# jarrodhroberson/diamond-types

Measured on AMD Instinct MI355X. Metric: merged ops/sec (whole node) for batched checkout, higher is better.
Workload: dtype u32/u8 integer

## Files before the change

diamond-types_amd/csrc/dt_replay.hip:

```cpp
#include <hip/hip_runtime.h>

#include <algorithm>
#include <cstdlib>
#include <stdint.h>

#include "dt_device.hpp"
#include "dt_wave.hpp"

namespace dtgpu {
namespace dev {
using namespace wave;

#define BALLOT(c) __ballot(c)
DEV uint32_t vflag(bool c) {
    uint32_t x = c ? 1u : 0u;
    asm volatile("" : "+v"(x));
    return x;
}

constexpr uint32_t BLK = 64;
constexpr uint32_t SBC = 64;
constexpr uint32_t ROOT_ID = 0xFFFFFFFFu;
constexpr uint32_t END_ID = 0xFFFFFFFEu;
constexpr uint32_t NONE = 0xFFFFFFFFu;
constexpr uint32_t C_VIS = 1u, C_LIVE = 1u << 8, C_ITEMS = 1u << 16;
constexpr uint32_t C_UP = 1u << 24;
constexpr uint32_t C_DIRTY = 1u << 31;
DEV uint32_t c_vis(uint32_t c) { return c & 0xFFu; }
DEV uint32_t c_live(uint32_t c) { return (c >> 8) & 0xFFu; }
DEV uint32_t c_items(uint32_t c) { return (c >> 16) & 0xFFu; }
DEV uint32_t c_up(uint32_t c) { return (c >> 24) & 0x7Fu; }
DEV uint32_t pc_blk(uint32_t w) { return w & 0xFFFFu; }
DEV uint32_t pc_cnt(uint32_t w) { return w >> 16; }
DEV uint32_t pc_of(uint32_t b, uint32_t k) { return b | (k << 16); }

template <typename T> DEV T ld(const T *p) { return *p; }
template <typename T> DEV T vld(const T *p) { return *reinterpret_cast<const volatile T *>(p); }
DEV const BatchParams &KP() {
    return *(const BatchParams *)(__builtin_amdgcn_kernarg_segment_ptr());
}
#define GLOBAL_AS __attribute__((address_space(1)))
template <typename T> DEV GLOBAL_AS T *gp(T *p) { return (GLOBAL_AS T *)p; }
template <typename T> DEV void st(T *p, T v) { *p = v; }
template <typename T> DEV T ld_sc(const T *p) { return __hip_atomic_load(p, __ATOMIC_RELAXED, __HIP_MEMORY_SCOPE_WORKGROUP); }
template <typename T> DEV void st_sc(T *p, T v) { __hip_atomic_store(p, v, __ATOMIC_RELAXED, __HIP_MEMORY_SCOPE_WORKGROUP); }
DEV uint32_t cv_add(uint32_t *p, uint32_t d) { return __hip_atomic_fetch_add(p, d, __ATOMIC_RELAXED, __HIP_MEMORY_SCOPE_WORKGROUP); }
template <typename T> DEV void at_xor(T *p, T v) { __hip_atomic_fetch_xor(p, v, __ATOMIC_RELAXED, __HIP_MEMORY_SCOPE_WORKGROUP); }
template <typename T> DEV void at_add(T *p, T v) { __hip_atomic_fetch_add(p, v, __ATOMIC_RELAXED, __HIP_MEMORY_SCOPE_WORKGROUP); }
template <typename T> DEV void at_or(T *p, T v) { __hip_atomic_fetch_or(p, v, __ATOMIC_RELAXED, __HIP_MEMORY_SCOPE_WORKGROUP); }

template <int L> DEV uint32_t ix(const uint32_t *p) {
    if (L) return *p;
    return ld_sc(p);
}
template <int L> DEV uint32_t ix16(const uint16_t *p) { return *p; }

enum ProfSlot { P_INS = 0, P_DEL, P_TOG, P_MAT, P_YJS, P_SPLIT, P_FIND, P_BLOAD, P_ORR, P_RUN, P_R1, P_R2, P_R3, P_N_YJS, P_N_SPLIT,
                P_T1, P_T2, P_T3, P_N_DIRTY, P_N_LOAD, P_N_LOOK, P_N_SKIP, P_N };

struct Doc {
    const Cmd *cmds;
    uint32_t ncmd, n_lv;
    const uint32_t *tlist;
    const DocDesc *desc;
    uint32_t *pc;
    u64 *ao;
    uint32_t *items;
    u64 *m2;
    uint32_t max_blocks, max_sb;
    uint32_t *cnt, *opos;
    uint16_t *opos16;
    uint32_t *sbn, *sbpos;
    uint32_t *top, *tlive;
    uint16_t *sbl;
    uint32_t nb, nsb;
    uint32_t err;
    uint32_t debug;
    uint32_t site;
    uint32_t steps;
    uint64_t prof[P_N];
    uint32_t doc;
    uint32_t cb, cit;
    u64 cmv, cml;
    uint32_t cpre, cpos;
    u64 *mup;
    uint32_t *tup;
    uint32_t *xf;
};

constexpr uint32_t PRE_NONE = 0x80000000u;
DEV bool pre_known(uint32_t pre) { return int32_t(pre) >= 0; }

DEV void fail(Doc &D, uint32_t code, uint32_t site) {
    if (!D.err) { D.err = code; D.site = site; }
}
DEV bool charge(Doc &D) {
    if (D.steps == 0) { fail(D, ErrCapacity, 1); return false; }
    D.steps--;
    return true;
}
template <bool PROF> DEV uint64_t tick() { return PROF ? __builtin_amdgcn_s_memtime() : 0; }

constexpr int IX_HBM = 0, IX_LDS = 1, IX_FLAT = 2;
template <int L> DEV uint32_t opos_of(const Doc &D, uint32_t b) {
    if (L) return D.opos16[b];
    return ix<L>(D.opos + b);
}
template <int L> DEV void set_opos(Doc &D, uint32_t b, uint32_t v) {
    if (L) D.opos16[b] = uint16_t(v);
    else D.opos[b] = v;
}


template <int L> DEV uint32_t first_block(const Doc &D) {
    if (L == IX_FLAT) return U(D.sbl[0]);
    return U(ix16<L>(D.sbl + size_t(U(ix<L>(D.top)) >> 16) * SBC));
}
template <int L> DEV uint32_t next_block(const Doc &D, uint32_t b) {
    if (L == IX_FLAT) {
        const uint32_t p = U(D.opos16[b]) + 1;
        return p < D.nb ? U(D.sbl[p]) : NONE;
    }
    const uint32_t o = U(opos_of<L>(D, b));
    const uint32_t S = o >> 6, i = o & 63u;
    if (i + 1 < U(ix<L>(D.sbn + S))) return U(ix16<L>(D.sbl + size_t(S) * SBC + i + 1));
    const uint32_t p = U(ix<L>(D.sbpos + S)) + 1;
    if (p >= D.nsb) return NONE;
    return U(ix16<L>(D.sbl + size_t(U(ix<L>(D.top + p)) >> 16) * SBC));
}
template <int L> DEV uint32_t key_at(const Doc &D, uint32_t b, uint32_t s) {
    if (L == IX_FLAT) return (uint32_t(D.opos16[b]) << 6) | s;
    const uint32_t o = opos_of<L>(D, b);
    return (ix<L>(D.sbpos + (o >> 6)) << 12) | ((o & 63u) << 6) | s;
}
DEV uint32_t find_slot(const Doc &D, uint32_t b, uint32_t item) {
    const uint4 *row = reinterpret_cast<const uint4 *>(D.items + size_t(b) * BLK);
    uint32_t s = BLK;
    for (uint32_t q = 0; q < BLK / 4 && s == BLK; q += 2) {
        uint4 v[2];
#pragma unroll
        for (uint32_t j = 0; j < 2; j++) v[j] = row[q + j];
#pragma unroll
        for (int j = 1; j >= 0; j--) {
            const uint32_t o = 4 * (q + uint32_t(j));
            if (v[j].w == item) s = o + 3;
            if (v[j].z == item) s = o + 2;
            if (v[j].y == item) s = o + 1;
            if (v[j].x == item) s = o;
        }
    }
    return s;
}
template <int L> DEV uint32_t key_of(const Doc &D, uint32_t item) {
    const uint32_t b = pc_blk(ld(D.pc + item));
    return key_at<L>(D, b, find_slot(D, b, item));
}
template <int L> DEV uint32_t ukey_of(const Doc &D, uint32_t item) {
    const uint32_t b = U(pc_blk(ld(D.pc + item)));
    const u64 m = BALLOT(D.items[size_t(b) * BLK + lane()] == item);
    return U(key_at<L>(D, b, ctz(m)));
}

struct Found {
    uint32_t b, k;
    uint32_t S, tp;
    uint32_t c;
    uint32_t p;
};
template <int L>
DEV bool find_vis(Doc &D, uint32_t p, Found &f) {
    const uint32_t l = lane();
    uint32_t base = 0, S = NONE;
    if (L == IX_FLAT) {
        const uint32_t nc = (D.nb + 63) >> 6;
        {
            const uint32_t w0 = D.top[min(l, nc - 1)];
            const uint32_t v = l < nc ? (w0 & 0xFFFFu) : 0u;
            const uint32_t inc = scan_incl32(v);
            const u64 m = BALLOT(inc > p) & 0xFFFFFFFFull;
            if (!m) return false;
            S = ctz(m);
            base = rdl(inc - v, S);
        }
        f.S = f.tp = S;
        const uint32_t q = (S << 6) + l;
        const uint32_t b0 = D.sbl[min(q, D.nb - 1)];
        const uint32_t w = D.cnt[b0];
        const uint32_t b = q < D.nb ? b0 : 0;
        const uint32_t v = q < D.nb ? c_vis(w) : 0;
        const uint32_t inc = scan_incl(v);
        const u64 m = BALLOT(base + inc > p);
        if (!m) return false;
        const uint32_t fl = ctz(m);
        f.b = U(rdl(b, fl));
        f.k = U(p - base - rdl(inc - v, fl));
        f.c = U(rdl(w, fl));
        f.p = (S << 6) + fl;
        return true;
    }
    for (uint32_t c = 0; c < D.nsb; c += 64) {
        const uint32_t i = c + l;
        const uint32_t w0 = ix<L>(D.top + min(i, D.nsb - 1));
        const uint32_t w = i < D.nsb ? w0 : 0;
        const uint32_t v = w & 0xFFFFu;
        const uint32_t inc = scan_incl(v);
        const u64 m = BALLOT(base + inc > p);
        if (m) {
            const uint32_t fl = ctz(m);
            S = U(rdl(w, fl) >> 16);
            f.tp = U(c + fl);
            base += rdl(inc - v, fl);
            break;
        }
        base += rdl(inc, 63);
    }
    if (S == NONE) return false;
    f.S = S;
    f.c = NONE;
    const uint32_t n = U(ix<L>(D.sbn + S));
    const uint32_t b0 = ix16<L>(D.sbl + size_t(S) * SBC + l);
    const uint32_t b = l < n ? b0 : 0;
    const uint32_t v0 = c_vis(ix<L>(D.cnt + b));
    const uint32_t v = l < n ? v0 : 0;
    const uint32_t inc = scan_incl(v);
    const u64 m = BALLOT(base + inc > p);
    if (!m) return false;
    const uint32_t fl = ctz(m);
    f.b = U(rdl(b, fl));
    f.k = U(p - base - rdl(inc - v, fl));
    return true;
}

DEV uint32_t select_bit(u64 m, uint32_t k) {
    const uint32_t l = lane();
    const bool set = (m >> l) & 1ull;
    const uint32_t before = uint32_t(__popcll(m & lanes_below(l)));
    return ctz(BALLOT(set && before == k));
}

template <int L>
DEV uint32_t next_live_block(Doc &D, uint32_t b) {
    const uint32_t l = lane();
    if (L == IX_FLAT) {
        const uint32_t p0 = U(D.opos16[b]) + 1, nc = (D.nb + 63) >> 6;
        uint32_t c = p0 >> 6;
        {
            const uint32_t q = (c << 6) + l;
            const uint32_t b0 = D.sbl[min(q, D.nb - 1)];
            const bool in = q >= p0 && q < D.nb;
            const uint32_t bl = in ? b0 : 0;
            const uint32_t cl = c_live(D.cnt[bl]);
            const u64 m = BALLOT(in && cl != 0);
            if (m) return U(rdl(bl, ctz(m)));
        }
        for (c = c + 1; c < nc; c += 64) {
            if (!charge(D)) return NONE;
            const uint32_t i = c + l;
            const uint32_t t = D.top[min(i, nc - 1)] >> 16;
            const u64 m = BALLOT(i < nc && t != 0);
            if (m) {
                const uint32_t q = ((c + ctz(m)) << 6) + l;
                const uint32_t b0 = D.sbl[min(q, D.nb - 1)];
                const uint32_t bl = q < D.nb ? b0 : 0;
                const uint32_t cl = c_live(D.cnt[bl]);
                const u64 m2 = BALLOT(q < D.nb && cl != 0);
                if (!m2) { fail(D, ErrCheckout, 19); return NONE; }
                return U(rdl(bl, ctz(m2)));
            }
        }
        return NONE;
    }
    const uint32_t o = U(opos_of<L>(D, b));
    uint32_t S = o >> 6;
    {
        const uint32_t n = U(ix<L>(D.sbn + S)), i0 = (o & 63u) + 1;
        const uint32_t b0 = ix16<L>(D.sbl + size_t(S) * SBC + l);
        const uint32_t bl = l < n ? b0 : 0;
        const uint32_t cl = c_live(ix<L>(D.cnt + bl));
        const u64 m = BALLOT(l >= i0 && l < n && cl != 0);
        if (m) return U(rdl(bl, ctz(m)));
    }
    for (uint32_t p = U(ix<L>(D.sbpos + S)) + 1; p < D.nsb; p += 64) {
        if (!charge(D)) return NONE;
        const uint32_t i = p + l;
        const uint32_t tl = ix<L>(D.tlive + min(i, D.nsb - 1));
        const u64 m = BALLOT(i < D.nsb && tl != 0);
        if (m) {
            S = U(ix<L>(D.top + p + ctz(m)) >> 16);
            const uint32_t n = U(ix<L>(D.sbn + S));
            const uint32_t b0 = ix16<L>(D.sbl + size_t(S) * SBC + l);
            const uint32_t bl = l < n ? b0 : 0;
            const uint32_t cl = c_live(ix<L>(D.cnt + bl));
            const u64 m2 = BALLOT(l < n && cl != 0);
            if (!m2) { fail(D, ErrCheckout, 19); return NONE; }
            return U(rdl(bl, ctz(m2)));
        }
    }
    return NONE;
}


template <int L, bool XF>
DEV void split_sb(Doc &D, uint32_t S) {
    const uint32_t l = lane();
    if (D.nsb >= D.max_sb) { fail(D, ErrCapacity, 21); return; }
    const uint32_t S2 = D.nsb;
    uint32_t vis = 0, live = 0, up = 0;
    {
        const uint32_t b = ix16<L>(D.sbl + size_t(S) * SBC + l);
        const uint32_t c = ix<L>(D.cnt + b);
        vis = c_vis(c);
        live = c_live(c);
        up = c_up(c);
        fence_wave();
        if (l >= SBC / 2) {
            D.sbl[size_t(S2) * SBC + (l - SBC / 2)] = uint16_t(b);
            set_opos<L>(D, b, (S2 << 6) | (l - SBC / 2));
        }
    }
    const uint32_t vh = wave_sum(l >= 32 ? vis : 0), lh = wave_sum(l >= 32 ? live : 0);
    const uint32_t vl = wave_sum(l < 32 ? vis : 0), ll = wave_sum(l < 32 ? live : 0);
    const uint32_t uh = XF ? wave_sum(l >= 32 ? up : 0) : 0, ul = XF ? wave_sum(l < 32 ? up : 0) : 0;
    const uint32_t p = U(ix<L>(D.sbpos + S)) + 1;
    for (int c = int(D.nsb) - 1; c >= int(p); c -= 64) {
        const int i = c - int(l);
        uint32_t w = 0, lv = 0, uv = 0;
        if (i >= int(p)) { w = ix<L>(D.top + i); lv = ix<L>(D.tlive + i); if (XF) uv = ix<L>(D.tup + i); }
        fence_wave();
        if (i >= int(p)) {
            D.top[i + 1] = w; D.tlive[i + 1] = lv; D.sbpos[w >> 16] = uint32_t(i + 1);
            if (XF) D.tup[i + 1] = uv;
        }
        fence_wave();
    }
    if (l == 0) {
        D.sbn[S] = SBC / 2;
        D.sbn[S2] = SBC / 2;
        D.top[p - 1] = (S << 16) | vl; D.tlive[p - 1] = ll;
        D.top[p] = (S2 << 16) | vh; D.tlive[p] = lh;
        D.sbpos[S2] = p;
        if (XF) { D.tup[p - 1] = ul; D.tup[p] = uh; }
    }
    fence_wave();
    D.nsb++;
}

template <int L, bool XF>
DEV uint32_t split_block(Doc &D, uint32_t b, uint32_t c, uint32_t it, u64 mv, u64 ml) {
    const uint32_t l = lane();
    if (D.nb >= D.max_blocks) { fail(D, ErrCapacity, 12); return 0; }
    const uint32_t b2 = D.nb;
    u64 mu = 0, mu_lo = 0, mu_hi = 0;
    if (XF) {
        mu = U64(ld(D.mup + b));
        mu_lo = mu & lanes_below(c);
        mu_hi = c >= 64 ? 0ull : mu >> c;
    }
    if (l >= c) {
        D.items[size_t(b2) * BLK + (l - c)] = it;
        st(D.pc + it, (ld(D.pc + it) & 0xFFFF0000u) | b2);
    }
    const u64 lo = lanes_below(c);
    const u64 mv_hi = c >= 64 ? 0ull : mv >> c, ml_hi = c >= 64 ? 0ull : ml >> c;
    if (l < 4) {
        const u64 v = l == 0 ? (mv & lo) : l == 1 ? (ml & lo) : l == 2 ? mv_hi : ml_hi;
        st(D.m2 + 2 * size_t(l < 2 ? b : b2) + (l & 1), v);
    }
    if (L == IX_FLAT) {
        const uint32_t pos = U(D.opos16[b]);
        for (int hi = int(D.nb) - 1; hi > int(pos); hi -= 64) {
            const int q = hi - int(l);
            const bool mvl = q > int(pos);
            uint32_t v = 0;
            if (mvl) v = D.sbl[q];
            fence_wave();
            if (mvl) {
                D.sbl[q + 1] = uint16_t(v);
                D.opos16[v] = uint16_t(q + 1);
                if (((q + 1) & 63) == 0) {
                    const uint32_t cv = D.cnt[v];
                    const uint32_t w = c_vis(cv) | (c_live(cv) << 16);
                    at_add(D.top + (uint32_t(q) >> 6), 0u - w);
                    at_add(D.top + (uint32_t(q + 1) >> 6), w);
                }
            }
            fence_wave();
        }
        if (l == 0) {
            const uint32_t v2 = uint32_t(__popcll(mv_hi)), l2 = uint32_t(__popcll(ml_hi));
            D.cnt[b2] = v2 * C_VIS + l2 * C_LIVE + (BLK - c) * C_ITEMS;
            D.cnt[b] = uint32_t(__popcll(mv & lo)) * C_VIS + uint32_t(__popcll(ml & lo)) * C_LIVE + c * C_ITEMS;
            D.sbl[pos + 1] = uint16_t(b2);
            D.opos16[b2] = uint16_t(pos + 1);
            if (((pos + 1) & 63) == 0) {
                const uint32_t w = v2 | (l2 << 16);
                at_add(D.top + (pos >> 6), 0u - w);
                at_add(D.top + ((pos + 1) >> 6), w);
            }
        }
        fence_wave();
        D.nb++;
        return b2;
    }
    const uint32_t o = U(opos_of<L>(D, b));
    const uint32_t S = o >> 6, i = o & 63u, n = U(ix<L>(D.sbn + S));
    {
        uint32_t v = 0;
        const bool mv_lane = l > i && l < n;
        if (mv_lane) v = ix16<L>(D.sbl + size_t(S) * SBC + l);
        fence_wave();
        if (mv_lane) {
            D.sbl[size_t(S) * SBC + l + 1] = uint16_t(v);
            set_opos<L>(D, v, (S << 6) | (l + 1));
        }
    }
    if (l == 0) {
        D.cnt[b2] = uint32_t(__popcll(mv_hi)) * C_VIS + uint32_t(__popcll(ml_hi)) * C_LIVE + (BLK - c) * C_ITEMS +
                    uint32_t(__popcll(mu_hi)) * C_UP;
        D.cnt[b] = uint32_t(__popcll(mv & lo)) * C_VIS + uint32_t(__popcll(ml & lo)) * C_LIVE + c * C_ITEMS +
                   uint32_t(__popcll(mu_lo)) * C_UP;
        if (XF) { st(D.mup + b, mu_lo); st(D.mup + b2, mu_hi); }
        D.sbl[size_t(S) * SBC + i + 1] = uint16_t(b2);
        set_opos<L>(D, b2, (S << 6) | (i + 1));
        D.sbn[S] = n + 1;
    }
    fence_wave();
    D.nb++;
    if (n + 1 == SBC) split_sb<L, XF>(D, S);
    return b2;
}

template <int L> DEV uint32_t cut_point(uint32_t s) { return L ? min(max(s, 16u), 48u) : BLK / 2; }

template <int L>
DEV uint32_t up_rank(Doc &D, uint32_t b, uint32_t s) {
    const uint32_t l = lane();
    const uint32_t o = U(opos_of<L>(D, b));
    const uint32_t S = o >> 6, i = o & 63u, tp = U(ix<L>(D.sbpos + S));
    uint32_t r = 0;
    for (uint32_t c = 0; c < tp; c += 64) r += wave_sum(c + l < tp ? ix<L>(D.tup + c + l) : 0u);
    const uint32_t bl = l < i ? ix16<L>(D.sbl + size_t(S) * SBC + l) : 0;
    r += wave_sum(l < i ? c_up(ix<L>(D.cnt + bl)) : 0u);
    r += uint32_t(__popcll(U64(ld(D.mup + b)) & lanes_below(s)));
    return U(r);
}

template <int L, bool PROF, bool XF>
DEV void insert_run(Doc &D, uint32_t b, uint32_t s, uint32_t it, u64 mv, u64 ml, uint32_t lv, uint32_t k,
                    uint32_t ol, uint32_t orr, uint32_t tph, uint32_t c_in) {
    constexpr bool PC = L == IX_FLAT && !XF;
    D.cb = NONE;
    const uint32_t b_in = b;
    const uint32_t l = lane();
    const uint32_t lv0 = lv, k0 = k;
    if (XF) {
        const uint32_t r0 = up_rank<L>(D, b, s);
        for (uint32_t j = l; j < k0; j += 64) D.xf[lv0 + j] = r0 + j;
    }
    if (!XF && c_in != NONE && c_items(c_in) + k <= BLK) {
        const uint32_t shifted = shfl(it, l >= k ? l - k : l);
        it = l < s ? it : (l < s + k ? lv + (l - s) : shifted);
        D.items[size_t(b) * BLK + l] = it;
        if (l >= s && l < s + k) st(D.pc + it, pc_of(b, 1u));
        const u64 low = lanes_below(s);
        const u64 ins = lanes_below(k) << s;
        mv = k == 64 ? ins : ((mv & low) | ((mv & ~low) << k) | ins);
        ml = k == 64 ? ins : ((ml & low) | ((ml & ~low) << k) | ins);
        st(D.m2 + 2 * size_t(b) + (l & 1u), (l & 1u) ? ml : mv);
        if (tph == NONE) tph = L == IX_FLAT ? U(uint32_t(D.opos16[b]) >> 6) : U(ix<L>(D.sbpos + (opos_of<L>(D, b) >> 6)));
        if (l == 0) {
            D.cnt[b] = c_in + k * (C_VIS + C_LIVE + C_ITEMS);
            if (L == IX_FLAT) {
                at_add(D.top + tph, k | (k << 16));
            } else {
                at_add(D.top + tph, k);
                at_add(D.tlive + tph, k);
            }
        }
        if (l < k) D.ao[lv + l] = u64(l == 0 ? ol : lv + l - 1) | (u64(orr) << 32);
        fence_wave();
        D.cb = b; D.cit = it; D.cmv = mv; D.cml = ml;
        return;
    }
    while (k > 0) {
        const uint32_t c = c_in != NONE ? c_in : U(ix<L>(D.cnt + b));
        c_in = NONE;
        const uint32_t bc = c_items(c);
        if (bc == BLK) {
            const uint64_t t0 = tick<PROF>();
            const uint32_t cut = cut_point<L>(s);
            const uint32_t b2 = split_block<L, XF>(D, b, cut, it, mv, ml);
            if (D.err) return;
            tph = NONE;
            if (s > cut || cut == BLK) {
                b = b2;
                s -= cut;
                it = shfl(it, (l + cut) & 63u);
                mv = cut >= 64 ? 0ull : mv >> cut;
                ml = cut >= 64 ? 0ull : ml >> cut;
            } else {
                mv &= lanes_below(cut);
                ml &= lanes_below(cut);
            }
            if (PROF) { D.prof[P_SPLIT] += tick<PROF>() - t0; D.prof[P_N_SPLIT]++; }
            continue;
        }
        uint64_t tr = tick<PROF>();
        const uint32_t m = min(k, BLK - bc);
        uint32_t *items = D.items + size_t(b) * BLK;
        const uint32_t shifted = shfl(it, l >= m ? l - m : l);
        it = l < s ? it : (l < s + m ? lv + (l - s) : shifted);
        items[l] = it;
        if (l >= s && l < s + m) st(D.pc + it, pc_of(b, 1u));
        if (PROF) { const uint64_t t = tick<PROF>(); D.prof[P_R1] += t - tr; tr = t; }
        const u64 low = lanes_below(s);
        const u64 ins = lanes_below(m) << s;
        mv = m == 64 ? ins : ((mv & low) | ((mv & ~low) << m) | ins);
        ml = m == 64 ? ins : ((ml & low) | ((ml & ~low) << m) | ins);
        st(D.m2 + 2 * size_t(b) + (l & 1u), (l & 1u) ? ml : mv);
        if (XF) {
            u64 mu = U64(ld(D.mup + b));
            mu = m == 64 ? ins : ((mu & low) | ((mu & ~low) << m) | ins);
            if (l == 0) st(D.mup + b, mu);
        }
        if (tph == NONE) tph = L == IX_FLAT ? U(uint32_t(D.opos16[b]) >> 6) : U(ix<L>(D.sbpos + (opos_of<L>(D, b) >> 6)));
        if (l == 0) {
            D.cnt[b] = c + m * (C_VIS + C_LIVE + C_ITEMS + (XF ? C_UP : 0u));
            const uint32_t tp = tph;
            if (L == IX_FLAT) {
                at_add(D.top + tp, m | (m << 16));
            } else {
                at_add(D.top + tp, m);
                at_add(D.tlive + tp, m);
            }
            if (XF) at_add(D.tup + tp, m);
        }
        fence_wave();
        if (PROF) { const uint64_t t = tick<PROF>(); D.prof[P_R2] += t - tr; tr = t; }
        lv += m;
        k -= m;
        s += m;
    }
    D.cb = b; D.cit = it; D.cmv = mv; D.cml = ml;
    if (PC && b != b_in) D.cpre = PRE_NONE;
    const uint64_t t3 = tick<PROF>();
    for (uint32_t j0 = 0; j0 < k0; j0 += 64) {
        const uint32_t j = j0 + l, nit = lv0 + j;
        if (j < k0) D.ao[nit] = u64(j == 0 ? ol : nit - 1) | (u64(orr) << 32);
    }
    if (PROF) D.prof[P_R3] += tick<PROF>() - t3;
}

DEV void agent_of(Doc &D, uint32_t lv, uint32_t &rank, uint32_t &seq) {
    const uint32_t l = lane();
    const GLOBAL_AS uint32_t *aruns = gp(vld(&KP().aruns)) + U(uint32_t(vld(&D.desc->arun_off)));
    uint32_t lo = 0, n = U(vld(&D.desc->n_aruns));
    while (n > 64) {
        if (!charge(D)) { rank = seq = 0; return; }
        const uint32_t stride = (n + 63) / 64;
        const uint32_t idx = lo + l * stride;
        const bool ok = l * stride < n && aruns[4 * idx] <= lv;
        const uint32_t k = uint32_t(__popcll(BALLOT(ok)));
        const uint32_t nlo = lo + (k ? k - 1 : 0) * stride;
        n = min(stride, lo + n - nlo);
        lo = nlo;
    }
    const bool ok = l < n && aruns[4 * (lo + l)] <= lv;
    const uint32_t k = uint32_t(__popcll(BALLOT(ok)));
    const uint32_t j = U(lo + (k ? k - 1 : 0));
    rank = U(aruns[4 * j + 1]);
    seq = U(aruns[4 * j + 2]) + (lv - U(aruns[4 * j]));
}

template <int L>
DEV void yjs_scan(Doc &D, uint32_t &b, uint32_t &s, uint32_t rb, uint32_t rs, uint32_t my_l, uint32_t my_r,
                  uint32_t ol_new, uint32_t orr_new, uint32_t lv) {
    const uint32_t l = lane();
    uint32_t new_rank, new_seq;
    agent_of(D, lv, new_rank, new_seq);
    bool scanning = false;
    uint32_t st_b = 0, st_s = 0;
    uint32_t cb = b, cs = s;
    for (;;) {
        if (!charge(D)) return;
        const uint32_t cnt = c_items(U(ix<L>(D.cnt + cb)));
        if (cs >= cnt) {
            const uint32_t nx = next_block<L>(D, cb);
            if (nx == NONE) break;
            cb = nx;
            cs = 0;
            continue;
        }
        const uint32_t end = cb == rb ? rs : cnt;
        if (cs >= end) break;
        const bool inr = l >= cs && l < end;
        const uint32_t o = l < cnt ? D.items[size_t(cb) * BLK + l] : 0;
        uint32_t ol_o = ROOT_ID, orr_o = END_ID;
        if (inr) {
            const u64 x = D.ao[o];
            ol_o = uint32_t(x);
            orr_o = uint32_t(x >> 32);
        }
        const uint32_t prev = shfl(o, (l - 1) & 63u);
        const bool l_eq = ol_o == ol_new, l_root = ol_o == ROOT_ID;
        const bool l_gt = !l_eq && !l_root && l > cs && ol_o == prev;
        uint32_t kl = l_eq ? my_l : (l_root ? 0u : (l_gt ? my_l + 1u : 0u));
        if (BALLOT(inr && !l_eq && !l_root && !l_gt)) {
            if (inr && !l_eq && !l_root && !l_gt) kl = key_of<L>(D, ol_o) + 1u;
        }
        uint32_t kr = 0xFFFFFFFFu;
        const bool need_r = inr && kl == my_l && orr_o != orr_new && orr_o != END_ID;
        if (BALLOT(need_r)) {
            if (need_r) kr = key_of<L>(D, orr_o);
        }
        const bool tie = inr && kl == my_l && orr_o == orr_new;
        bool new_lt = false;
        for (u64 mt = BALLOT(tie); mt; mt &= mt - 1) {
            const uint32_t f = ctz(mt);
            uint32_t r2, s2;
            agent_of(D, U(rdl(o, f)), r2, s2);
            const bool lt = new_rank < r2 || (new_rank == r2 && new_seq < s2);
            if (l == f) new_lt = lt;
        }
        const bool stop = inr && (kl < my_l || (tie && new_lt));
        const bool setv = inr && kl == my_l && orr_o != orr_new && kr < my_r;
        const bool clr = inr && kl == my_l && !stop && !setv;
        const u64 ms = BALLOT(stop);
        const uint32_t lim = ms ? ctz(ms) : end;
        const u64 below = lanes_below(lim);
        const u64 mset = BALLOT(setv) & below, mclr = BALLOT(clr) & below;
        if (mset | mclr) {
            const int lc = mclr ? int(last_lane(mclr)) : -1;
            const int ls = mset ? int(last_lane(mset)) : -1;
            if (ls > lc) {
                const u64 after = lc >= 0 ? (mset & ~((2ull << lc) - 1ull)) : mset;
                if (lc >= 0 || !scanning) { scanning = true; st_b = cb; st_s = ctz(after); }
            } else {
                scanning = false;
            }
        }
        cs = lim;
        if (ms) break;
    }
    if (scanning) { b = st_b; s = st_s; }
    else { b = cb; s = cs; }
    b = U(b);
    s = U(s);
}

template <int L, bool PROF = false>
DEV void load_block(Doc &D, uint32_t b, uint32_t c, uint32_t &it, u64 &mv, u64 &ml) {
    const uint32_t l = lane();
    const uint32_t bc = c_items(c);
    if (PROF) { D.prof[P_N_LOAD]++; if (c & C_DIRTY) D.prof[P_N_DIRTY]++; }
    const uint32_t it0 = D.items[size_t(b) * BLK + l];
    it = l < bc ? it0 : 0;
    if (c & C_DIRTY) {
        const uint32_t k = pc_cnt(ld(D.pc + it));
        mv = BALLOT(l < bc && k == 1u);
        ml = BALLOT(l < bc && k != 0u);
        st(D.m2 + 2 * size_t(b) + (l & 1u), (l & 1u) ? ml : mv);
        if (l == 0) D.cnt[b] = c & ~C_DIRTY;
        fence_wave();
    } else {
        const u64 x = ld(D.m2 + 2 * size_t(b) + (l & 1u));
        mv = rdl64(x, 0);
        ml = rdl64(x, 1);
    }
}

template <int L, bool PROF, bool XF>
DEV void do_insert(Doc &D, uint32_t lv, uint32_t k, uint32_t pos) {
    uint64_t tp = tick<PROF>();
    uint32_t b, kk = 0, tph = 0;
    uint32_t fcnt = NONE;
    constexpr bool PC = L == IX_FLAT && !XF;
    if (pos == 0) {
        b = first_block<L>(D);
        if (PC) { D.cpre = 0; D.cpos = 0; }
    } else {
        const uint32_t rk = pos - 1 - D.cpre;
        const uint32_t hit = PC ? U(uint32_t(rk < uint32_t(__popcll(D.cmv)))) : 0u;
        if (hit) {
            b = D.cb;
            kk = rk;
            tph = D.cpos >> 6;
        } else {
            Found f;
            if (!find_vis<L>(D, pos - 1, f)) { fail(D, ErrCheckout, 13); return; }
            b = f.b;
            kk = f.k;
            tph = f.tp;
            fcnt = f.c;
            if (PC) { D.cpre = pos - 1 - f.k; D.cpos = f.p; }
        }
        if (PC && PROF) D.prof[P_N_SKIP] += hit;
    }
    if (PC && PROF) D.prof[P_N_LOOK]++;
    if (PROF) { const uint64_t t = tick<PROF>(); D.prof[P_FIND] += t - tp; tp = t; }
    const uint32_t c0 = L == IX_FLAT && fcnt != NONE ? fcnt : U(ix<L>(D.cnt + b));
    const uint32_t bc = c_items(c0);
    uint32_t cb = c0 & ~C_DIRTY;
    uint32_t it;
    u64 mv, ml;
    if (b == D.cb) { it = D.cit; mv = D.cmv; ml = D.cml; }
    else load_block<L, PROF>(D, b, c0, it, mv, ml);
    uint32_t s = 0, ol = ROOT_ID;
    if (pos) {
        const uint32_t s0 = select_bit(mv, kk);
        if (s0 >= bc) { fail(D, ErrCheckout, 13); return; }
        ol = U(rdl(it, s0));
        s = s0 + 1;
    }
    if (PROF) { const uint64_t t = tick<PROF>(); D.prof[P_BLOAD] += t - tp; tp = t; }
    const u64 mlr = s >= 64 ? 0ull : (ml & (~0ull << s));
    uint32_t rb, rs, orr;
    bool direct;
    if (mlr) {
        rb = b;
        rs = ctz(mlr);
        orr = U(rdl(it, rs));
        direct = rs == s;
    } else {
        rb = next_live_block<L>(D, b);
        if (D.err) return;
        if (rb != NONE) {
            uint32_t rit;
            u64 rmv, rml;
            load_block<L, PROF>(D, rb, U(ix<L>(D.cnt + rb)), rit, rmv, rml);
            rs = ctz(rml);
            orr = U(rdl(rit, rs));
        } else {
            rs = 0;
            orr = END_ID;
        }
        if (s < bc) direct = false;
        else {
            const uint32_t nx = next_block<L>(D, b);
            direct = nx == NONE || (rb == nx && rs == 0);
        }
    }
    if (PROF) { const uint64_t t = tick<PROF>(); D.prof[P_ORR] += t - tp; tp = t; }
    if (!direct) {
        const uint32_t my_l = ol == ROOT_ID ? 0u : ukey_of<L>(D, ol) + 1u;
        const uint32_t my_r = orr == END_ID ? 0xFFFFFFFFu : ukey_of<L>(D, orr);
        const uint32_t b0 = b;
        yjs_scan<L>(D, b, s, rb, rs, my_l, my_r, ol, orr, lv);
        if (D.err) return;
        if (b != b0) {
            cb = U(ix<L>(D.cnt + b));
            if (b == D.cb) { it = D.cit; mv = D.cmv; ml = D.cml; }
            else load_block<L, PROF>(D, b, cb, it, mv, ml);
            cb &= ~C_DIRTY;
            tph = NONE;
            if (PC) D.cpre = PRE_NONE;
        }
        if (PROF) { const uint64_t t = tick<PROF>(); D.prof[P_YJS] += t - tp; tp = t; D.prof[P_N_YJS]++; }
    }
    const uint64_t sp0 = PROF ? D.prof[P_SPLIT] : 0;
    insert_run<L, PROF, XF>(D, b, s, it, mv, ml, lv, k, ol, orr, tph, cb);
    if (PROF) D.prof[P_RUN] += tick<PROF>() - tp - (D.prof[P_SPLIT] - sp0);
}

template <int L, bool PROF, bool XF>
DEV void do_delete(Doc &D, uint32_t lv, uint32_t n, uint32_t pos, bool fwd) {
    const uint32_t l = lane();
    uint32_t j0 = 0;
    uint32_t up_done = 0;
    while (j0 < n) {
        constexpr bool PC = L == IX_FLAT && !XF;
        Found f;
        const uint32_t rk = pos - D.cpre;
        const uint32_t hit = PC ? U(uint32_t(rk < uint32_t(__popcll(D.cmv)))) : 0u;
        if (hit) {
            f.b = D.cb;
            f.k = rk;
            f.tp = D.cpos >> 6;
            f.c = NONE;
        } else {
            if (!find_vis<L>(D, pos, f)) { fail(D, ErrCheckout, 14); return; }
            if (PC) { D.cpre = pos - f.k; D.cpos = f.p; }
        }
        if (PC && PROF) { D.prof[P_N_LOOK]++; D.prof[P_N_SKIP] += hit; }
        const uint32_t b = f.b, kk = f.k, tpos = f.tp;
        const uint32_t c0 = L == IX_FLAT && f.c != NONE ? f.c : U(ix<L>(D.cnt + b));
        uint32_t it;
        u64 mv, ml;
        if (b == D.cb) { it = D.cit; mv = D.cmv; ml = D.cml; }
        else load_block<L, PROF>(D, b, c0, it, mv, ml);
        const uint32_t c = c0 & ~C_DIRTY;
        const uint32_t avail = c_vis(c) - kk;
        const uint32_t take = min(avail, n - j0);
        const uint32_t r = uint32_t(__popcll(mv & lanes_below(l)));
        const bool sel = ((mv >> l) & 1ull) && r >= kk && r < kk + take;
        const u64 selm = BALLOT(sel);
        if (uint32_t(__popcll(selm)) != take || take == 0) { fail(D, ErrCheckout, 15); return; }
        u64 mu = 0;
        uint32_t base = 0;
        if (XF) {
            mu = U64(ld(D.mup + b));
            base = up_rank<L>(D, b, 0);
        }
        if (sel) {
            const uint32_t j = j0 + (r - kk);
            const uint32_t dlv = fwd ? lv + j : lv + n - 1 - j;
            st(D.pc + it, pc_of(b, 2u));
            *reinterpret_cast<uint32_t *>(D.ao + dlv) = it;
            if (XF) {
                const u64 below = lanes_below(l);
                const uint32_t x = fwd ? base + uint32_t(__popcll(mu & ~selm & below))
                                       : base + uint32_t(__popcll(mu & below)) + up_done;
                D.xf[dlv] = ((mu >> l) & 1ull) ? x : NONE;
            }
        }
        const uint32_t gone = XF ? uint32_t(__popcll(mu & selm)) : 0u;
        up_done += gone;
        if (l == 0) {
            st(D.m2 + 2 * size_t(b), mv & ~selm);
            D.cnt[b] = c - take * C_VIS - gone * C_UP;
            at_add(D.top + tpos, 0u - take);
            if (XF) {
                st(D.mup + b, mu & ~selm);
                D.tup[tpos] = ix<L>(D.tup + tpos) - gone;
            }
        }
        fence_wave();
        D.cb = b; D.cit = it; D.cmv = mv & ~selm; D.cml = ml;
        j0 += take;
    }
}

template <int L, bool PROF>
DEV void toggle_pass(Doc &D, uint32_t off, uint32_t n, uint32_t pre, bool have_pre) {
    const uint32_t l = lane();
    uint64_t tq = tick<PROF>();
    auto resolve = [&](uint32_t j, uint32_t e, uint32_t &item, bool &del, bool &bad) {
        const bool valid = j + l < n;
        const uint32_t lv = e & 0x3FFFFFFFu;
        bad = valid && lv >= D.n_lv;
        del = valid && !bad && ((e >> 30) & 1u);
        const uint32_t tgt = *reinterpret_cast<const uint32_t *>(D.ao + (del ? lv : 0u));
        item = valid ? (del ? tgt : lv) : 0u;
    };
    if (n == 0) return;
    const uint32_t last = off + n - 1;
    uint32_t e_cur = have_pre ? pre : D.tlist[min(off + l, last)];
    uint32_t e_nx = 0;
    if (n > 64) e_nx = D.tlist[min(off + 64 + l, last)];
    uint32_t it_cur;
    bool del_cur, bad_cur;
    resolve(0, e_cur, it_cur, del_cur, bad_cur);
    for (uint32_t j = 0; j < n; j += 64) {
        bool bad = bad_cur || it_cur >= D.n_lv;
        bool act = j + l < n && !bad;
        const bool del = del_cur;
        const uint32_t item = it_cur;
        int32_t d = int32_t((e_cur >> 31) << 1) - 1;
        int32_t dneg = int32_t(e_cur >> 31) - 1;
        if (j + 64 < n) {
            e_cur = e_nx;
            resolve(j + 64, e_cur, it_cur, del_cur, bad_cur);
            e_nx = D.tlist[min(off + j + 128 + l, last)];
        }
        if (BALLOT(bad)) { fail(D, ErrCheckout, 16); return; }
        if (PROF) { const uint64_t t = tick<PROF>(); D.prof[P_T1] += t - tq; tq = t; }
        const u64 dmask = BALLOT(act && del);
        bool dup = del;
        if (__popcll(dmask) > 4) {
            dup = false;
            const uint32_t x = act ? item : (0x80000000u | l);
            uint32_t r0 = x, r1 = shfl(x, (l + 16) & 63u), r2 = shfl(x, (l + 32) & 63u), r3 = shfl(x, (l + 48) & 63u);
            uint32_t mn = min(min(r1 ^ x, r2 ^ x), r3 ^ x);
#pragma unroll
            for (int k = 1; k < 16; k++) {
                r0 = uint32_t(__builtin_amdgcn_mov_dpp(int(r0), 0x13C, 0xF, 0xF, false));
                r1 = uint32_t(__builtin_amdgcn_mov_dpp(int(r1), 0x13C, 0xF, 0xF, false));
                r2 = uint32_t(__builtin_amdgcn_mov_dpp(int(r2), 0x13C, 0xF, 0xF, false));
                r3 = uint32_t(__builtin_amdgcn_mov_dpp(int(r3), 0x13C, 0xF, 0xF, false));
                mn = min(mn, min(min(r0 ^ x, r1 ^ x), min(r2 ^ x, r3 ^ x)));
            }
            dup = mn == 0u;
        }
        for (u64 dm = BALLOT(act && dup); dm;) {
            const uint32_t t = rdl(item, ctz(dm));
            const u64 same = BALLOT(act && item == t);
            if (__popcll(same) > 1) {
                const bool mine = (same >> l) & 1ull;
                const int32_t sum = int32_t(wave_sum(mine ? uint32_t(d) : 0u));
                const int32_t neg = int32_t(wave_sum(mine ? uint32_t(dneg) : 0u));
                if (mine) {
                    if (l == ctz(same)) { d = sum; dneg = neg; }
                    else act = false;
                }
            }
            dm &= ~same;
        }
        bool fv = false, fl = false;
        uint32_t b = 0;
        int32_t dv = 0, dl = 0;
        {
            const uint32_t w = ld(D.pc + (act ? item : 0u));
            const uint32_t bw = pc_blk(w), oc = pc_cnt(w), nc = oc + uint32_t(d);
            const bool badc = act && int32_t((oc + uint32_t(dneg)) | (0xFFFFu - nc) | (D.nb - 1u - bw)) < 0;
            const bool ok = act && !badc;
            bad = bad || badc;
            if (ok) st(D.pc + item, pc_of(bw, nc));
            b = ok ? bw : 0u;
            fv = ok && ((oc == 1) != (nc == 1));
            fl = ok && ((oc != 0) != (nc != 0));
            dv = fv ? (nc == 1 ? 1 : -1) : 0;
// ... 430 lines not shown
    }
    len_out = total;
    items_out = items;
}

template <int L, bool XF>
DEV uint32_t check_invariants(Doc &D, DocResult *res) {
    const uint32_t l = lane();
    const uint32_t n_ids = D.n_lv;
    uint32_t blocks = 0;
    const uint32_t nlists = L == IX_FLAT ? (D.nb + 63) >> 6 : D.nsb;
    for (uint32_t p = 0; p < nlists; p++) {
        uint32_t S = p, n;
        if (L == IX_FLAT) {
            n = min(64u, D.nb - 64 * p);
        } else {
            S = U(ix<L>(D.top + p)) >> 16;
            if (U(ix<L>(D.sbpos + S)) != p) return 205;
            n = U(ix<L>(D.sbn + S));
            if (n == 0 || n >= SBC) return 206;
        }
        uint32_t tv = 0, tl = 0, tu = 0;
        for (uint32_t i = 0; i < n; i++) {
            const uint32_t b = U(ix16<L>(D.sbl + size_t(S) * (L == IX_FLAT ? 64u : SBC) + i));
            if (U(opos_of<L>(D, b)) != (L == IX_FLAT ? 64 * p + i : ((S << 6) | i))) return 201;
            const uint32_t c = U(ix<L>(D.cnt + b));
            const uint32_t cnt = c_items(c);
            const bool dirty = (c & C_DIRTY) != 0;
            u64 mv = U64(ld(D.m2 + 2 * size_t(b))), ml = U64(ld(D.m2 + 2 * size_t(b) + 1));
            if (dirty) {
                const uint32_t i2 = l < cnt ? D.items[size_t(b) * BLK + l] : 0;
                const uint32_t k = l < cnt && i2 < n_ids ? pc_cnt(ld(D.pc + i2)) : 0u;
                mv = BALLOT(l < cnt && k == 1u);
                ml = BALLOT(l < cnt && k != 0u);
            }
            if (uint32_t(__popcll(mv)) != c_vis(c) || uint32_t(__popcll(ml)) != c_live(c)) return 207;
            if (XF && uint32_t(__popcll(U64(ld(D.mup + b)))) != c_up(c)) return 209;
            if (XF) tu += c_up(c);
            tv += c_vis(c);
            tl += c_live(c);
            bool bad = false;
            uint32_t w = 0, it = 0xFFFFFFFFu;
            if (l < cnt) {
                it = D.items[size_t(b) * BLK + l];
                if (it >= n_ids) bad = true;
                else {
                    w = pc_blk(ld(D.pc + it));
                    const uint32_t k = pc_cnt(ld(D.pc + it));
                    if (((mv >> l) & 1) != (k == 1 ? 1u : 0u)) bad = true;
                    if (((ml >> l) & 1) != (k != 0 ? 1u : 0u)) bad = true;
                    if (w != b || find_slot(D, b, it) != l) bad = true;
                }
            } else if (((mv | ml) >> l) & 1) bad = true;
            const u64 bm = BALLOT(bad);
            if (bm) {
                if (l == ctz(bm)) {
                    res->dbg[0] = b; res->dbg[1] = l; res->dbg[2] = cnt; res->dbg[3] = it; res->dbg[4] = w;
                    res->dbg[5] = uint32_t(mv); res->dbg[6] = uint32_t(mv >> 32);
                    res->dbg[7] = uint32_t(ml); res->dbg[8] = uint32_t(ml >> 32);
                }
                return 202;
            }
            blocks++;
        }
        if (tv != (U(ix<L>(D.top + p)) & 0xFFFFu)) return 203;
        if (tl != (L == IX_FLAT ? U(ix<L>(D.top + p)) >> 16 : U(ix<L>(D.tlive + p)))) return 204;
        if (XF && tu != U(ix<L>(D.tup + p))) return 210;
    }
    if (blocks != D.nb) return 208;
    if (L == IX_FLAT) {
        for (uint32_t c = nlists + l; c < D.max_sb; c += 64)
            if (BALLOT(D.top[c] != 0)) return 211;
    }
    if (L == IX_FLAT && !XF && D.cb != NONE && pre_known(D.cpre)) {
        if (D.cb >= D.nb || U(D.opos16[D.cb]) != D.cpos) return 212;
        uint32_t before = 0;
        for (uint32_t q0 = 0; q0 < D.cpos; q0 += 64) {
            const uint32_t q = q0 + l;
            before += wave_sum(q < D.cpos ? c_vis(D.cnt[D.sbl[min(q, D.nb - 1)]]) : 0u);
        }
        if (U(before) != D.cpre) return 212;
        if (uint32_t(__popcll(D.cmv)) != c_vis(U(D.cnt[D.cb]))) return 213;
    }
    return 0;
}

template <int L, bool PROF, bool XF, bool MW>
DEV void run_doc(Doc &D) {
    const uint32_t l = lane();
    D.nb = 1;
    D.nsb = 1;
    D.err = 0;
    D.site = 0;
    const uint32_t seg_lo = U(vld(&D.desc->seg_lo)), seg_hi = U(vld(&D.desc->seg_hi));
    if (!XF && (seg_lo != 0 || seg_hi != NONE)) {
        const uint32_t c0 = seg_lo ? U(seg_cmd(D.cmds, D.ncmd, seg_lo)) : 0u;
        const uint32_t c1 = seg_hi != NONE ? U(seg_cmd(D.cmds, D.ncmd, seg_hi)) : D.ncmd;
        if (c1 < c0 || seg_straddles(D.cmds, c0, seg_lo) || seg_straddles(D.cmds, c1, seg_hi)) fail(D, ErrCheckout, 30);
        else { D.cmds += c0; D.ncmd = c1 - c0; }
    }
    D.steps = uint32_t(min<uint64_t>(64ull * (uint64_t(D.ncmd) + D.n_lv) + 4096, 0xFFFFFFF0ull));
    const uint32_t seg_u = XF ? 0u : U(vld(&D.desc->seg_u));
    if (seg_u) {
        if (!D.err) init_phantoms<L>(D, seg_u);
    } else {
        if (L == IX_FLAT) {
            for (uint32_t c = l; c < D.max_sb; c += 64) D.top[c] = 0;
            if (l == 0) { D.cnt[0] = 0; D.opos16[0] = 0; D.sbl[0] = 0; }
        } else if (l == 0) {
            D.cnt[0] = 0; set_opos<L>(D, 0, 0);
            D.sbl[0] = 0; D.sbn[0] = 1; D.sbpos[0] = 0; D.top[0] = 0; D.tlive[0] = 0;
            if (XF) { D.tup[0] = 0; st(D.mup, 0ull); }
        }
        if (l < 2) st(D.m2 + l, 0ull);
        fence_wave();
    }
    D.cb = NONE;
    D.cit = 0;
    D.cmv = D.cml = 0;
    D.cpre = PRE_NONE;
    D.cpos = 0;
    if (PROF) for (int i = 0; i < P_N; i++) D.prof[i] = 0;
    const uint64_t t_start = tick<PROF>();
    uint32_t pf = 0;
    bool pf_ok = false;
    uint32_t ci = 0;
    for (uint32_t base = 0; base < D.ncmd && !D.err; base += 64) {
        const uint32_t n_here = min(64u, D.ncmd - base);
        Cmd pre = {0, 0, 0, 0};
        pre = D.cmds[min(base + l, D.ncmd - 1)];
        const uint32_t op_l = pre.op & 15u;
        const bool apply_l = op_l == CMD_INS || op_l == CMD_DEL;
        const u64 bad_cmds = BALLOT(l < n_here && (op_l > CMD_TOG || (apply_l && (pre.len == 0 || pre.lv >= D.n_lv ||
                                                                               pre.len > D.n_lv - pre.lv))));
        const u64 tog_cmds = BALLOT(l < n_here && op_l == CMD_TOG);
        const uint32_t n_ok = bad_cmds ? ctz(bad_cmds) : n_here;
        for (uint32_t j = 0; j < n_ok && !D.err; j++) {
            ci = base + j;
            const uint32_t op = U(rdl(pre.op, j)), a = U(rdl(pre.lv, j)), n = U(rdl(pre.len, j)),
                           pos = U(rdl(pre.pos, j));
            uint32_t nx_pf = 0;
            bool nx_ok = false;
            if ((tog_cmds >> j) & 2ull) {
                const uint32_t o2 = U(rdl(pre.lv, j + 1)), n2 = U(rdl(pre.len, j + 1));
                if (n2) nx_pf = D.tlist[o2 + min(l, n2 - 1)];
                nx_ok = true;
            }
            const uint64_t t0 = tick<PROF>();
            if ((op & 15u) == CMD_INS) {
                do_insert<L, PROF, XF>(D, a, n, pos);
                if (PROF) D.prof[P_INS] += tick<PROF>() - t0;
            } else if ((op & 15u) == CMD_DEL) {
                do_delete<L, PROF, XF>(D, a, n, pos, (op & 16u) != 0);
                if (PROF) D.prof[P_DEL] += tick<PROF>() - t0;
            } else {
                if (MW && n >= TOG_MW_MIN) toggle_mw<L>(D, a, n);
                else if (n <= 64) toggle_pass_1<L, PROF>(D, a, n, pf, pf_ok);
                else toggle_pass<L, PROF>(D, a, n, pf, pf_ok);
                if (PROF) D.prof[P_TOG] += tick<PROF>() - t0;
            }
            if (PROF && (D.debug & 1u) && !D.err) {
                const uint32_t code = check_invariants<L, XF>(D, vld(&KP().results) + D.doc);
                if (code) fail(D, ErrCheckout, code);
            }
            pf = nx_pf;
            pf_ok = nx_ok;
        }
        if (bad_cmds && !D.err) {
            ci = base + n_ok;
            fail(D, ErrCheckout, (U(rdl(pre.op, n_ok)) & 15u) > CMD_TOG ? 18u : 17u);
        }
    }
    if (L && D.err == ErrCapacity && (D.site == 12 || D.site == 21)) {
        uint32_t *fb_list = vld(&KP().fb_list);
        if (fb_list) {
            if (l == 0) gp(fb_list)[atomicAdd(vld(&KP().fb_count), 1u)] = D.doc;
            return;
        }
    }
    uint32_t len = 0, n_items = 0;
    u64 h = 0;
    const uint64_t t_mat = tick<PROF>();
    if (!D.err) {
        const uint64_t so = vld(&D.desc->src_off);
        if (!XF && so != ~0ull) {
            const uint32_t cap = U(vld(&D.desc->src_cap));
            materialise_src<L>(D, gp(vld(&KP().src)) + so, cap, len, n_items);
            if (len > cap) { fail(D, ErrCapacity, 32); len = 0; }
        } else {
            GLOBAL_AS uint8_t *out = gp(vld(&KP().out)) + vld(&D.desc->out_off);
            materialise<L>(D, out, U(vld(&D.desc->out_cap)), len, h, n_items);
        }
    }
    GLOBAL_AS DocResult *res = gp(vld(&KP().results)) + D.doc;
    if (l == 0) {
        res->status = D.err;
        res->out_len = len;
        res->hash = h;
        res->n_items = n_items;
        res->n_blocks = D.nb;
        res->n_sb = D.nsb;
        res->lds = L ? 1u : 0u;
// ... 259 lines not shown
```

Baseline: 10.25 billion.

## Pack visible/live flags into per-lane item registers instead of wave masks

Moves the per-block visible and live state from two wave-uniform 64-bit masks into the high bits of each lane's item id, rebuilding the masks with ballots when needed. Mask shift and merge arithmetic in insert and split paths is replaced by per-lane selects, and the cached live mask is dropped from the doc state. This trades scalar 64-bit bit manipulation for extra ballots and masking of ids on every use. It also adds a capacity check limiting ids below bit 30 and a new cached-state consistency check.

Result: faster. 10.46 billion (median of 6 runs) (+2.1%).

```diff
diff --git a/diamond-types_amd/csrc/dt_replay.hip b/diamond-types_amd/csrc/dt_replay.hip
--- a/diamond-types_amd/csrc/dt_replay.hip
+++ b/diamond-types_amd/csrc/dt_replay.hip
@@ -33,6 +33,10 @@
 DEV uint32_t pc_blk(uint32_t w) { return w & 0xFFFFu; }
 DEV uint32_t pc_cnt(uint32_t w) { return w >> 16; }
 DEV uint32_t pc_of(uint32_t b, uint32_t k) { return b | (k << 16); }
+constexpr uint32_t F_LIVE = 1u << 31, F_VIS = 1u << 30, ID_MASK = F_VIS - 1u;
+DEV bool f_vis(uint32_t it) { return it >= (F_LIVE | F_VIS); }
+DEV bool f_live(uint32_t it) { return int32_t(it) < 0; }
+DEV uint32_t f_of_count(uint32_t k) { return k == 1u ? (F_LIVE | F_VIS) : (k ? F_LIVE : 0u); }
 
 template <typename T> DEV T ld(const T *p) { return *p; }
 template <typename T> DEV T vld(const T *p) { return *reinterpret_cast<const volatile T *>(p); }
@@ -81,7 +85,7 @@
     uint64_t prof[P_N];
     uint32_t doc;
     uint32_t cb, cit;
-    u64 cmv, cml;
+    u64 cmv;
     uint32_t cpre, cpos;
     u64 *mup;
     uint32_t *tup;
@@ -231,11 +235,9 @@
     return true;
 }
 
-DEV uint32_t select_bit(u64 m, uint32_t k) {
-    const uint32_t l = lane();
-    const bool set = (m >> l) & 1ull;
-    const uint32_t before = uint32_t(__popcll(m & lanes_below(l)));
-    return ctz(BALLOT(set && before == k));
+DEV uint32_t select_vis(uint32_t it, u64 mv, uint32_t k) {
+    const uint32_t rank = f_vis(it) ? bits_below(mv) : NONE;
+    return uint32_t(__ffsll(BALLOT(rank == k)) - 1);
 }
 
 template <int L>
@@ -346,10 +348,12 @@
 }
 
 template <int L, bool XF>
-DEV uint32_t split_block(Doc &D, uint32_t b, uint32_t c, uint32_t it, u64 mv, u64 ml) {
+DEV uint32_t split_block(Doc &D, uint32_t b, uint32_t c, uint32_t itf) {
     const uint32_t l = lane();
     if (D.nb >= D.max_blocks) { fail(D, ErrCapacity, 12); return 0; }
     const uint32_t b2 = D.nb;
+    const uint32_t it = itf & ID_MASK;
+    const u64 mv = BALLOT(f_vis(itf)), ml = BALLOT(f_live(itf));
     u64 mu = 0, mu_lo = 0, mu_hi = 0;
     if (XF) {
         mu = U64(ld(D.mup + b));
@@ -446,7 +450,7 @@
 }
 
 template <int L, bool PROF, bool XF>
-DEV void insert_run(Doc &D, uint32_t b, uint32_t s, uint32_t it, u64 mv, u64 ml, uint32_t lv, uint32_t k,
+DEV void insert_run(Doc &D, uint32_t b, uint32_t s, uint32_t it, uint32_t lv, uint32_t k,
                     uint32_t ol, uint32_t orr, uint32_t tph, uint32_t c_in) {
     constexpr bool PC = L == IX_FLAT && !XF;
     D.cb = NONE;
@@ -459,13 +463,11 @@
     }
     if (!XF && c_in != NONE && c_items(c_in) + k <= BLK) {
         const uint32_t shifted = shfl(it, l >= k ? l - k : l);
-        it = l < s ? it : (l < s + k ? lv + (l - s) : shifted);
-        D.items[size_t(b) * BLK + l] = it;
-        if (l >= s && l < s + k) st(D.pc + it, pc_of(b, 1u));
-        const u64 low = lanes_below(s);
-        const u64 ins = lanes_below(k) << s;
-        mv = k == 64 ? ins : ((mv & low) | ((mv & ~low) << k) | ins);
-        ml = k == 64 ? ins : ((ml & low) | ((ml & ~low) << k) | ins);
+        const uint32_t j = l - s;
+        it = l < s ? it : (j < k ? (lv + j) | F_LIVE | F_VIS : shifted);
+        D.items[size_t(b) * BLK + l] = it & ID_MASK;
+        if (j < k) st(D.pc + (lv + j), pc_of(b, 1u));
+        const u64 mv = BALLOT(f_vis(it)), ml = BALLOT(f_live(it));
         st(D.m2 + 2 * size_t(b) + (l & 1u), (l & 1u) ? ml : mv);
         if (tph == NONE) tph = L == IX_FLAT ? U(uint32_t(D.opos16[b]) >> 6) : U(ix<L>(D.sbpos + (opos_of<L>(D, b) >> 6)));
         if (l == 0) {
@@ -479,7 +481,7 @@
         }
         if (l < k) D.ao[lv + l] = u64(l == 0 ? ol : lv + l - 1) | (u64(orr) << 32);
         fence_wave();
-        D.cb = b; D.cit = it; D.cmv = mv; D.cml = ml;
+        D.cb = b; D.cit = it; D.cmv = mv;
         return;
     }
     while (k > 0) {
@@ -489,18 +491,16 @@
         if (bc == BLK) {
             const uint64_t t0 = tick<PROF>();
             const uint32_t cut = cut_point<L>(s);
-            const uint32_t b2 = split_block<L, XF>(D, b, cut, it, mv, ml);
+            const uint32_t b2 = split_block<L, XF>(D, b, cut, it);
             if (D.err) return;
             tph = NONE;
             if (s > cut || cut == BLK) {
                 b = b2;
                 s -= cut;
-                it = shfl(it, (l + cut) & 63u);
-                mv = cut >= 64 ? 0ull : mv >> cut;
-                ml = cut >= 64 ? 0ull : ml >> cut;
+                const uint32_t up = shfl(it, (l + cut) & 63u);
+                it = l + cut < BLK ? up : 0u;
             } else {
-                mv &= lanes_below(cut);
-                ml &= lanes_below(cut);
+                it = l < cut ? it : 0u;
             }
             if (PROF) { D.prof[P_SPLIT] += tick<PROF>() - t0; D.prof[P_N_SPLIT]++; }
             continue;
@@ -509,16 +509,16 @@
         const uint32_t m = min(k, BLK - bc);
         uint32_t *items = D.items + size_t(b) * BLK;
         const uint32_t shifted = shfl(it, l >= m ? l - m : l);
-        it = l < s ? it : (l < s + m ? lv + (l - s) : shifted);
-        items[l] = it;
-        if (l >= s && l < s + m) st(D.pc + it, pc_of(b, 1u));
+        const uint32_t j = l - s;
+        it = l < s ? it : (j < m ? (lv + j) | F_LIVE | F_VIS : shifted);
+        items[l] = it & ID_MASK;
+        if (j < m) st(D.pc + (lv + j), pc_of(b, 1u));
         if (PROF) { const uint64_t t = tick<PROF>(); D.prof[P_R1] += t - tr; tr = t; }
-        const u64 low = lanes_below(s);
-        const u64 ins = lanes_below(m) << s;
-        mv = m == 64 ? ins : ((mv & low) | ((mv & ~low) << m) | ins);
-        ml = m == 64 ? ins : ((ml & low) | ((ml & ~low) << m) | ins);
+        const u64 mv = BALLOT(f_vis(it)), ml = BALLOT(f_live(it));
         st(D.m2 + 2 * size_t(b) + (l & 1u), (l & 1u) ? ml : mv);
         if (XF) {
+            const u64 low = lanes_below(s);
+            const u64 ins = lanes_below(m) << s;
             u64 mu = U64(ld(D.mup + b));
             mu = m == 64 ? ins : ((mu & low) | ((mu & ~low) << m) | ins);
             if (l == 0) st(D.mup + b, mu);
@@ -541,7 +541,7 @@
         k -= m;
         s += m;
     }
-    D.cb = b; D.cit = it; D.cmv = mv; D.cml = ml;
+    D.cb = b; D.cit = it; D.cmv = BALLOT(f_vis(it));
     if (PC && b != b_in) D.cpre = PRE_NONE;
     const uint64_t t3 = tick<PROF>();
     for (uint32_t j0 = 0; j0 < k0; j0 += 64) {
@@ -649,7 +649,7 @@
 }
 
 template <int L, bool PROF = false>
-DEV void load_block(Doc &D, uint32_t b, uint32_t c, uint32_t &it, u64 &mv, u64 &ml) {
+DEV void load_block(Doc &D, uint32_t b, uint32_t c, uint32_t &it, u64 &mv) {
     const uint32_t l = lane();
     const uint32_t bc = c_items(c);
     if (PROF) { D.prof[P_N_LOAD]++; if (c & C_DIRTY) D.prof[P_N_DIRTY]++; }
@@ -657,15 +657,17 @@
     it = l < bc ? it0 : 0;
     if (c & C_DIRTY) {
         const uint32_t k = pc_cnt(ld(D.pc + it));
-        mv = BALLOT(l < bc && k == 1u);
-        ml = BALLOT(l < bc && k != 0u);
+        it |= l < bc ? f_of_count(k) : 0u;
+        mv = BALLOT(f_vis(it));
+        const u64 ml = BALLOT(f_live(it));
         st(D.m2 + 2 * size_t(b) + (l & 1u), (l & 1u) ? ml : mv);
         if (l == 0) D.cnt[b] = c & ~C_DIRTY;
         fence_wave();
     } else {
         const u64 x = ld(D.m2 + 2 * size_t(b) + (l & 1u));
         mv = rdl64(x, 0);
-        ml = rdl64(x, 1);
+        const u64 ml = rdl64(x, 1);
+        it |= (uint32_t(mv >> l) & 1u) << 30 | (uint32_t(ml >> l) & 1u) << 31;
     }
 }
 
@@ -702,34 +704,34 @@
     const uint32_t bc = c_items(c0);
     uint32_t cb = c0 & ~C_DIRTY;
     uint32_t it;
-    u64 mv, ml;
-    if (b == D.cb) { it = D.cit; mv = D.cmv; ml = D.cml; }
-    else load_block<L, PROF>(D, b, c0, it, mv, ml);
+    u64 mv;
+    if (b == D.cb) { it = D.cit; mv = D.cmv; }
+    else load_block<L, PROF>(D, b, c0, it, mv);
     uint32_t s = 0, ol = ROOT_ID;
     if (pos) {
-        const uint32_t s0 = select_bit(mv, kk);
+        const uint32_t s0 = select_vis(it, mv, kk);
         if (s0 >= bc) { fail(D, ErrCheckout, 13); return; }
-        ol = U(rdl(it, s0));
+        ol = U(rdl(it, s0)) & ID_MASK;
         s = s0 + 1;
     }
     if (PROF) { const uint64_t t = tick<PROF>(); D.prof[P_BLOAD] += t - tp; tp = t; }
-    const u64 mlr = s >= 64 ? 0ull : (ml & (~0ull << s));
+    const u64 mlr = BALLOT((uint32_t(int32_t(it) >> 31) & (lane() + 1u)) > s);
     uint32_t rb, rs, orr;
     bool direct;
     if (mlr) {
         rb = b;
         rs = ctz(mlr);
-        orr = U(rdl(it, rs));
+        orr = U(rdl(it, rs)) & ID_MASK;
         direct = rs == s;
     } else {
         rb = next_live_block<L>(D, b);
         if (D.err) return;
         if (rb != NONE) {
             uint32_t rit;
-            u64 rmv, rml;
-            load_block<L, PROF>(D, rb, U(ix<L>(D.cnt + rb)), rit, rmv, rml);
-            rs = ctz(rml);
-            orr = U(rdl(rit, rs));
+            u64 rmv;
+            load_block<L, PROF>(D, rb, U(ix<L>(D.cnt + rb)), rit, rmv);
+            rs = ctz(BALLOT(f_live(rit)));
+            orr = U(rdl(rit, rs)) & ID_MASK;
         } else {
             rs = 0;
             orr = END_ID;
@@ -749,8 +751,8 @@
         if (D.err) return;
         if (b != b0) {
             cb = U(ix<L>(D.cnt + b));
-            if (b == D.cb) { it = D.cit; mv = D.cmv; ml = D.cml; }
-            else load_block<L, PROF>(D, b, cb, it, mv, ml);
+            if (b == D.cb) { it = D.cit; mv = D.cmv; }
+            else load_block<L, PROF>(D, b, cb, it, mv);
             cb &= ~C_DIRTY;
             tph = NONE;
             if (PC) D.cpre = PRE_NONE;
@@ -758,7 +760,7 @@
         if (PROF) { const uint64_t t = tick<PROF>(); D.prof[P_YJS] += t - tp; tp = t; D.prof[P_N_YJS]++; }
     }
     const uint64_t sp0 = PROF ? D.prof[P_SPLIT] : 0;
-    insert_run<L, PROF, XF>(D, b, s, it, mv, ml, lv, k, ol, orr, tph, cb);
+    insert_run<L, PROF, XF>(D, b, s, it, lv, k, ol, orr, tph, cb);
     if (PROF) D.prof[P_RUN] += tick<PROF>() - tp - (D.prof[P_SPLIT] - sp0);
 }
 
@@ -785,14 +787,14 @@
         const uint32_t b = f.b, kk = f.k, tpos = f.tp;
         const uint32_t c0 = L == IX_FLAT && f.c != NONE ? f.c : U(ix<L>(D.cnt + b));
         uint32_t it;
-        u64 mv, ml;
-        if (b == D.cb) { it = D.cit; mv = D.cmv; ml = D.cml; }
-        else load_block<L, PROF>(D, b, c0, it, mv, ml);
+        u64 mv;
+        if (b == D.cb) { it = D.cit; mv = D.cmv; }
+        else load_block<L, PROF>(D, b, c0, it, mv);
         const uint32_t c = c0 & ~C_DIRTY;
         const uint32_t avail = c_vis(c) - kk;
         const uint32_t take = min(avail, n - j0);
-        const uint32_t r = uint32_t(__popcll(mv & lanes_below(l)));
-        const bool sel = ((mv >> l) & 1ull) && r >= kk && r < kk + take;
+        const uint32_t r = bits_below(mv);
+        const bool sel = (f_vis(it) ? r - kk : NONE) < take;
         const u64 selm = BALLOT(sel);
         if (uint32_t(__popcll(selm)) != take || take == 0) { fail(D, ErrCheckout, 15); return; }
         u64 mu = 0;
@@ -804,8 +806,8 @@
         if (sel) {
             const uint32_t j = j0 + (r - kk);
             const uint32_t dlv = fwd ? lv + j : lv + n - 1 - j;
-            st(D.pc + it, pc_of(b, 2u));
-            *reinterpret_cast<uint32_t *>(D.ao + dlv) = it;
+            st(D.pc + (it & ID_MASK), pc_of(b, 2u));
+            *reinterpret_cast<uint32_t *>(D.ao + dlv) = it & ID_MASK;
             if (XF) {
                 const u64 below = lanes_below(l);
                 const uint32_t x = fwd ? base + uint32_t(__popcll(mu & ~selm & below))
@@ -825,7 +827,7 @@
             }
         }
         fence_wave();
-        D.cb = b; D.cit = it; D.cmv = mv & ~selm; D.cml = ml;
+        D.cb = b; D.cit = sel ? it & ~F_VIS : it; D.cmv = mv & ~selm;
         j0 += take;
     }
 }
@@ -1422,6 +1424,14 @@
         if (U(before) != D.cpre) return 212;
         if (uint32_t(__popcll(D.cmv)) != c_vis(U(D.cnt[D.cb]))) return 213;
     }
+    if (D.cb != NONE) {
+        if (D.cb >= D.nb) return 214;
+        const uint32_t cnt = c_items(U(ix<L>(D.cnt + D.cb)));
+        const uint32_t i2 = l < cnt ? D.items[size_t(D.cb) * BLK + l] : 0u;
+        const uint32_t k = l < cnt && i2 < n_ids ? pc_cnt(ld(D.pc + i2)) : 0u;
+        const uint32_t want = l < cnt ? (i2 | f_of_count(k)) : 0u;
+        if (BALLOT(D.cit != want) || BALLOT(f_vis(D.cit)) != D.cmv) return 214;
+    }
     return 0;
 }
 
@@ -1432,6 +1442,7 @@
     D.nsb = 1;
     D.err = 0;
     D.site = 0;
+    if (D.n_lv >= F_VIS || D.n_lv < U(vld(&D.desc->n_lv))) fail(D, ErrCapacity, 33);
     const uint32_t seg_lo = U(vld(&D.desc->seg_lo)), seg_hi = U(vld(&D.desc->seg_hi));
     if (!XF && (seg_lo != 0 || seg_hi != NONE)) {
         const uint32_t c0 = seg_lo ? U(seg_cmd(D.cmds, D.ncmd, seg_lo)) : 0u;
@@ -1457,7 +1468,7 @@
     }
     D.cb = NONE;
     D.cit = 0;
-    D.cmv = D.cml = 0;
+    D.cmv = 0;
     D.cpre = PRE_NONE;
     D.cpos = 0;
     if (PROF) for (int i = 0; i < P_N; i++) D.prof[i] = 0;
```
